# mbitsnbites/himg

Hardware: AMD Instinct MI355X
Metric: Mpixels/s encode+decode, 4K RGBA q=50 (higher is better)
Workload: dtype u8/i16/i32 integer

## Files before the change

### himg_amd/csrc/kernels_dec.hip

```cpp
#include "himg_dev.h"
#include "loop_counts.h"

#include <cstdlib>
#include <type_traits>

namespace himg_dev {

__device__ static constexpr uint8_t kScanD[64] = {
    0,  1,  9,  8,  16, 17, 18, 10, 2,  3,  11, 19, 27, 26, 25, 24,
    32, 33, 34, 35, 36, 28, 20, 12, 4,  5,  13, 21, 29, 37, 45, 44,
    43, 42, 41, 40, 48, 49, 50, 51, 52, 53, 54, 46, 38, 30, 22, 14,
    6,  7,  15, 23, 31, 39, 47, 55, 63, 62, 61, 60, 59, 58, 57, 56};

__device__ static constexpr uint8_t kInvScanD[64] = {
    0, 1, 8, 9, 24, 25, 48, 49, 3, 2, 7, 10, 23, 26, 47, 50, 4, 5, 6, 11, 22, 27, 46, 51, 15, 14, 13, 12, 21, 28, 45, 52, 16, 17, 18, 19, 20, 29, 44, 53, 35, 34, 33, 32, 31, 30, 43, 54, 36, 37, 38, 39, 40, 41, 42, 55, 63, 62, 61, 60, 59, 58, 57, 56};

constexpr int kStGeom = 1, kStUnsupported = 3, kStFormat = 4;
__device__ __host__ constexpr int fmt_err(int stage, int huff) { return kStFormat | (stage << 4) | (huff << 8); }
constexpr int kMaxDepth = 32;
constexpr int kMaxNodes = 2 * kNumSym - 1;
constexpr int kMaxSlow = 128;

__device__ __forceinline__ int clamp255d(int x) { return x < 0 ? 0 : (x > 255 ? 255 : x); }

// ... 1147 lines not shown
      if (__builtin_expect(y == 0, 0)) {
        if ((by >> 31) && tm == TM) {
          ntm = ((1u << (by & 255u)) - 1u) << 3;
          ntb = TB + (((1u << kLutBits) + ((by >> 8) & 0xffffu)) << 3);
          y = (uint32_t)kLutBits | ((uint32_t)kLutBits << 27);
          by = 0;
        } else {
          const int base = tm == TM ? 0 : kLutBits;
          uint32_t len;
          y = walk_token(rd, tb, by, base, &len, &by, &bad);
          adv = len - (uint32_t)base;
        }
      }
      tm = ntm; tbase = ntb;
      const uint32_t extra = __builtin_amdgcn_ubfe((uint32_t)rd.win, y, y >> 5);
      const uint32_t n = y >> 27;
      rd.consume((int)n);
      put(by);
      o += ((y >> 10) & 511u) + extra;
      bp += adv + n;
    };
    while ((int)bp <= limk) step();
    if (tm != TM) step();
    while (bp < lim) {
      uint32_t nbits, cnt, by;
      lean_step<true>(rd, tb, true, &nbits, &cnt, &by, &bad);
      put(by);
      o += cnt;
      bp += nbits;
    }
    rd.retire();
    if (bad) sh->err = 1;
    return;
  }
  for (;;) {
    uint32_t nbits, cnt, by;
    lean_step<true>(rd, tb, exact || (int)bp > limk, &nbits, &cnt, &by, &bad);
    if (exact && (bad || op + cnt > out_size)) { bad = true; break; }
    if (by) {
      if (op + 4 <= op_end) {
        asm volatile("global_store_dword %0, %1, %2" :: "v"((uint32_t)op), "v"(by), "s"(gout) : "memory");
      } else {
#pragma unroll
        for (int j = 0; j < 4; ++j) {
          const uint32_t b = (by >> (8 * j)) & 255u;
          if (b) gout[op + j] = (uint8_t)b;
        }
      }
    }
    op += cnt;
    bp += nbits;
    if (exact && op >= out_size) { sh->endbit = endbit_base + (bp - rel0); break; }
    if (!(bp < lim)) break;
  }
  rd.retire();
  if (bad) sh->err = 1;
}

constexpr uint32_t kTailBits = 48;
struct SubGrid {
  uint32_t b0, lim;
  bool active;
  int last_active;
};
__device__ __forceinline__ SubGrid sub_grid(uint32_t rel0, uint32_t bits, uint32_t sb, int tid) {
  SubGrid q;
  const uint32_t la = (bits - 1u) / sb, L = bits - la * sb;
  const uint32_t S = (L > kTailBits && la + 1u < (uint32_t)kDecThreads) ? sb - (L - kTailBits) : 0u;
  const uint32_t rel_end = rel0 + bits;
  q.b0 = tid ? rel0 + (uint32_t)tid * sb - S : rel0;
  q.lim = rel0 + (uint32_t)(tid + 1) * sb - S;
  if (q.lim > rel_end) q.lim = rel_end;
  q.active = q.b0 < rel_end;
  q.last_active = (int)((bits - 1u + S) / sb);
  return q;
}

struct PreLane {
  uint32_t start, off, nxt, tot, endrel, valid, rounds;
  uint32_t nstart;
};

struct ColdFix { uint32_t start, endpos, cnt, rounds; unsigned long long off, tot; long long c_first; };
__device__ __attribute__((noinline)) ColdFix cold_fixpoint(const uint8_t *p, uint32_t stream_size,
                                                           unsigned long long abs_bit, const uint32_t *grp_lds,
                                                           const uint32_t *nd_lds, StreamShared *sh, bool active,
                                                           uint32_t lim, uint32_t start, uint32_t lead_bits) {
  GrpTables tb;
  tb.grp = reinterpret_cast<const uint2 *>(grp_lds); tb.gx = nullptr; tb.gy = nullptr; tb.nd = nd_lds;
  GReader rd;
  const uint32_t rel0 = rd.attach(p, stream_size, abs_bit);
  ColdFix r;
  r.start = start; r.endpos = start; r.cnt = 0; r.rounds = 0; r.c_first = 0;
  lean_fixpoint(rd, tb, sh, rel0, active, lim, &r.start, &r.endpos, &r.cnt, &r.rounds, false, lead_bits, &r.c_first);
  r.off = block_scan_u64(r.cnt, sh->sm64, &r.tot);
  return r;
}

template <bool FUSED, bool GLOBAL = false, bool PRIMED = false>
__device__ __forceinline__ int decode_stream(const uint8_t *p, uint32_t stream_size, uint32_t pay_off,
                             uint32_t pay_len, uint32_t out_size, const GrpTables &tb,
                             StreamShared *sh, uint8_t *lds_out, uint32_t *win, uint8_t *gout,
                             uint32_t *stats, uint32_t max_sub, uint32_t lead_bits,
                             const uint32_t *pre_start = nullptr, const uint32_t *pre_off = nullptr) {
  const int tid = threadIdx.x;
  if (!PRIMED) {
    if (tid == 0) { sh->err = 0; sh->endbit = ~0ull; }
    __syncthreads();
  }

  const unsigned long long P1 = 8ull * pay_len;
  unsigned long long cur = 0;
  unsigned long long O0 = 0;
  uint32_t st_chunks = 0, st_rounds = 0;
  long long c_sync = 0, c_write = 0, c_r1 = 0, c_t0 = clock64();
  bool synced = false;

  while (cur < P1 && O0 < out_size) {
    synced = false;
    GReader rd;
    const uint32_t rel0 = rd.attach(p, stream_size, 8ull * pay_off + cur);
    ++st_chunks;

    const unsigned long long rem = P1 - cur;
    uint32_t sub = (uint32_t)((rem + kDecThreads - 1) / kDecThreads);
    sub = (sub + 31u) & ~31u;
    sub = sub < kMinSubBits ? kMinSubBits : (sub > max_sub ? max_sub : sub);
    const unsigned long long chunk_bits = (unsigned long long)sub * kDecThreads;
    const uint32_t rel_end = rel0 + (uint32_t)(rem < chunk_bits ? rem : chunk_bits);
    const SubGrid sg = sub_grid(rel0, rel_end - rel0, sub, tid);
    const uint32_t my_b0 = sg.b0, lim = sg.lim;
    const bool active = sg.active;
    const int last_active = sg.last_active;

    uint32_t start = active ? my_b0 : rel_end, endpos = start, cnt = 0;
    unsigned long long tot, off;
    uint32_t wlim = lim;
    const uint32_t pre_valid = cur != 0 ? 0u : pre_off ? pre_off[kDecThreads + 2] : 0u;
    const bool pre = pre_valid != 0, chain = pre_valid == 3u;
    if (pre) {
      const uint32_t ns = tid + 1 < kDecThreads ? pre_start[tid + 1] : ~0u;
      wlim = ns < rel_end - rel0 ? rel0 + ns : rel_end;
    }
    if (pre) {
      start = rel0 + pre_start[tid];
      off = pre_off[tid];
      const uint32_t nxt_off = pre_off[tid + 1];
      cnt = nxt_off - (uint32_t)off;
      tot = pre_off[kDecThreads];
      if (tid == last_active) endpos = rel0 + pre_off[kDecThreads + 1];
      st_rounds += pre_off[kDecThreads + 3];
    } else {
      const ColdFix cf = cold_fixpoint(p, stream_size, 8ull * pay_off + cur, reinterpret_cast<const uint32_t *>(tb.grp),
                                       tb.nd, sh, active, lim, start, lead_bits);
      start = cf.start; endpos = cf.endpos; cnt = cf.cnt; st_rounds += cf.rounds;
      c_r1 += cf.c_first; off = cf.off; tot = cf.tot;
    }
    { const long long t = clock64(); c_sync += t - c_t0; c_t0 = t; }

    const unsigned long long opl = O0 + off;
    const bool inside = opl + cnt < out_size, exact = !inside && opl < out_size;
    if (FUSED) {
      uint32_t end_bp = ~0u;
      if (inside) {
        if (!lean_write(rd, tb, start, wlim, (uint32_t)opl, lds_out, 0u, chain)) sh->err = 1;
      } else if (exact) {
        if (!exact_write(rd, tb, start, wlim, (uint32_t)opl, out_size, lds_out, &end_bp)) sh->err = 1;
      }
      if (end_bp != ~0u) sh->endbit = cur + (end_bp - rel0);
      __syncthreads();
    } else if (GLOBAL) {
      lean_write_global(rd, tb, sh, start, wlim, opl, exact, out_size, cur, rel0, gout, exact ? opl : opl + cnt);
      __syncthreads();
    } else {
      const unsigned long long O1 = (O0 + tot < out_size) ? O0 + tot : out_size;
      lean_write_windows(rd, tb, sh, start, wlim, opl, exact, O0, O1, out_size, cur, rel0, win, gout);
    }
    { const long long t = clock64(); c_write += t - c_t0; c_t0 = t; }

    if (tid == last_active) sh->nxt[0] = endpos;
    __syncthreads();
    const uint32_t last_end = sh->nxt[0];
    cur += (unsigned long long)(last_end - rel0);
    O0 += tot;
    if (last_end == rel0) break;
    __syncthreads();
  }
  if (!synced) __syncthreads();

  int bad = sh->err;
  if (O0 < out_size) bad = 1;
  const unsigned long long E = sh->endbit;
  if (!bad && !(E <= P1 && E + 8 > P1 && E > 0)) bad = 1;
  if (tid == 0 && stats) {
    stats[0] = st_chunks; stats[1] = st_rounds;
    if (!FUSED) { stats[2] = 0; stats[3] = (uint32_t)(c_r1 >> 4); }
    stats[4] = (uint32_t)(c_sync >> 4); stats[5] = (uint32_t)(c_write >> 4);
    stats[6] = pay_len; stats[7] = out_size;
  }
  return bad;
}

__device__ __forceinline__ int decode_row_recorded(const uint8_t *p, uint32_t stream_size, uint32_t pay_off,
                                                   uint32_t pay_len, uint32_t out_size, const GrpTables &tb,
                                                   StreamShared *sh, uint8_t *lds_out, uint32_t *stats,
                                                   const PreLane &pl) {
  const int tid = threadIdx.x;
  const unsigned long long P1 = 8ull * pay_len;
  if (pl.valid == 0 || P1 == 0 || out_size == 0) return -1;
  const long long c_t0 = clock64();
  GReader rd;
  const uint32_t rel0 = rd.attach(p, stream_size, 8ull * pay_off);
  const uint32_t rel_end = rel0 + (uint32_t)P1;
  const uint32_t start = rel0 + pl.start, opl = pl.off, cnt = pl.nxt - pl.off;
  const uint32_t wlim = pl.nstart < (uint32_t)P1 ? rel0 + pl.nstart : rel_end;
  const bool inside = opl + cnt < out_size, exact = !inside && opl < out_size;
  uint32_t end_bp = ~0u;
  if (inside) {
    if (!lean_write(rd, tb, start, wlim, opl, lds_out, 0u, pl.valid == 3u)) sh->err = 1;
  } else if (exact) {
    if (!exact_write(rd, tb, start, wlim, opl, out_size, lds_out, &end_bp)) sh->err = 1;
  }
  if (end_bp != ~0u) sh->endbit = (unsigned long long)(end_bp - rel0);
  __syncthreads();
  const long long c_t1 = clock64();
  int bad = sh->err;
  if (pl.tot < out_size) bad = 1;
  const unsigned long long E = sh->endbit;
  if (!bad && !(E <= P1 && E + 8 > P1 && E > 0)) bad = 1;
  if (tid == 0 && stats) {
    stats[0] = 1; stats[1] = pl.rounds;
    stats[4] = 0; stats[5] = (uint32_t)((c_t1 - c_t0) >> 4);
    stats[6] = pay_len; stats[7] = out_size;
  }
  return bad;
}

// ... 86 lines not shown
  stage_payload(gr, s_pay, (uint32_t)kLresPayWords);
  __syncthreads();
  rd.w = (const __attribute__((address_space(3))) uint32_t *)s_pay;
  rd.jmax = kLresPayWords - 1;
  const unsigned long long rem = P1 - cur;
  const uint32_t rel_end = rel0 + (uint32_t)(rem < (unsigned long long)kLresChunkBits ? rem : kLresChunkBits);
  const uint32_t my_b0 = rel0 + tid * kLresSubBits;
  uint32_t lim = my_b0 + kLresSubBits;
  if (lim > rel_end) lim = rel_end;
  const bool active = my_b0 < rel_end;
  const int last_active = (int)((rel_end - rel0 - 1u) / kLresSubBits);
  uint32_t start = active ? my_b0 : rel_end, endpos = start, cnt = 0, rounds = 0, first = rel0;
  if (FIX) {
    const unsigned long long T = ws.spec_end[slot - 1];
    if (T < cur || T >= cur + kLresSubBits) {
      if (tid == 0) ws.fix_end[slot] = ~0ull;
      return;
    }
    first = rel0 + (uint32_t)(T - cur);
    start = rel0 + ws.spec_start[slot * kDecThreads + tid];
    endpos = rel0 + ws.spec_endpos[slot * kDecThreads + tid];
    cnt = ws.spec_cnt[slot * kDecThreads + tid];
  }
  uint32_t memo[3 * kLresMemo];
  uint32_t *gm = ws.spec_memo + (slot * kDecThreads + tid) * kLresMemo;
#pragma unroll
  for (int e = 0; e < kLresMemo; ++e) {
    memo[3 * e] = ~0u; memo[3 * e + 1] = memo[3 * e + 2] = 0;
    if (FIX && tid > 0) {
      const uint32_t m = gm[e];
      if (m != ~0u) { memo[3 * e] = my_b0 + (m & 63u); memo[3 * e + 1] = lim + ((m >> 6) & 63u); memo[3 * e + 2] = m >> 12; }
    }
  }
  const long long c_in = clock64();
  lean_fixpoint<false, LReader, kLresMemo>(rd, tb, sh, first, active, lim, &start, &endpos, &cnt, &rounds, FIX,
                                           (uint32_t)g.lead_bits, nullptr, nullptr, memo);
  const long long c_fix = clock64() - c_in;
  if (!FIX) {
#pragma unroll
    for (int e = 0; e < kLresMemo; ++e) {
      const uint32_t ds = memo[3 * e] - my_b0, de = memo[3 * e + 1] - lim;
      gm[e] = (memo[3 * e] == ~0u || tid == 0 || ds > 46u || de > 46u || memo[3 * e + 2] >= (1u << 20))
                  ? ~0u : (ds | (de << 6) | (memo[3 * e + 2] << 12));
    }
  }
  unsigned long long tot;
  block_scan_u64(cnt, sh->sm64, &tot);
  ws.spec_start[slot * kDecThreads + tid] = start - rel0;
  ws.spec_endpos[slot * kDecThreads + tid] = endpos - rel0;
  ws.spec_cnt[slot * kDecThreads + tid] = cnt;
  if (tid == last_active) { end_out[slot] = cur + (endpos - rel0); ws.spec_tot[slot] = tot; }
  if (tid == 0) {
    uint32_t *st = ws.stats + ((size_t)f * (g.rows + 1)) * 8;
    atomicAdd(&st[FIX ? 2 : 0], 1u);
    atomicAdd(&st[FIX ? 3 : 1], rounds);
    atomicMax(&st[FIX ? 5 : 4], rounds);
    atomicMax(&st[FIX ? 7 : 6], (uint32_t)(c_fix >> 4));
  }
}

__global__ __launch_bounds__(kDecThreads) void k_lres_spec(Geom g, DecWs ws, const uint8_t *packed,
                                                           size_t in_stride, const uint32_t *sizes) {
  __shared__ LdsTables T;
  __shared__ StreamShared sh;
  __shared__ __attribute__((aligned(16))) uint32_t s_pay[kLresPayWords];
  const int k = blockIdx.x, f = blockIdx.y, tid = threadIdx.x;
  DecFrame *df = ws.frames + f;
  if (tid == 0) sh.flag = df->status;
  __syncthreads();
  if (sh.flag) return;
  const unsigned long long P1 = 8ull * (df->s[0].chunk_end - df->s[0].payload_off);
  const unsigned long long cur = (unsigned long long)k * kLresChunkBits;
  const size_t slot = (size_t)f * ws.lres_chunks + k;
  if (cur >= P1) {
    if (tid == 0) { ws.spec_end[slot] = cur; ws.spec_tot[slot] = 0; }
    return;
  }
  load_dec_tables(ws, df, f, 0, &T);
  __syncthreads();
  const GrpTables tb = tables_of(&T);
  lres_chain_body<false>(g, ws, packed + (size_t)f * in_stride, sizes[f], df, f, k, tb, &sh, s_pay);
}

__global__ __launch_bounds__(kDecThreads) void k_lres_fix(Geom g, DecWs ws, const uint8_t *packed,
                                                          size_t in_stride, const uint32_t *sizes) {
  __shared__ LdsTables T;
  __shared__ StreamShared sh;
  __shared__ uint8_t s_pending[kDecThreads];
  __shared__ int s_bad;
  __shared__ __attribute__((aligned(16))) uint32_t s_pay[kLresPayWords];
  const int f = blockIdx.x, k = threadIdx.x;
  DecFrame *df = ws.frames + f;
  if (k == 0) { ws.ver_ok[f] = 0; ws.lres_endbit[f] = ~0ull; s_bad = 0; sh.flag = df->status; }
  s_pending[k] = 0;
  __syncthreads();
  if (sh.flag) return;
  const uint32_t pay_off = df->s[0].payload_off;
  const unsigned long long P1 = 8ull * (df->s[0].chunk_end - pay_off);
  const int nact = (int)((P1 + kLresChunkBits - 1) / kLresChunkBits);
  if (nact > ws.lres_chunks || nact > kDecThreads) return;
  load_dec_tables(ws, df, f, 0, &T);
  __syncthreads();
  const GrpTables tb = tables_of(&T);
  const uint8_t *p = packed + (size_t)f * in_stride;
  const size_t slot = (size_t)f * ws.lres_chunks + k;
  const unsigned long long cur = (unsigned long long)k * kLresChunkBits;
  if (k == 0) {
    ws.fix_end[slot] = ws.spec_end[slot];
  } else if (k < nact) {
    const unsigned long long T = ws.spec_end[slot - 1];
    bool settled = false;
    if (T >= cur && T < cur + kLresSubBits) {
      GReader rd;
      const uint32_t rel0 = rd.attach(p, sizes[f], 8ull * pay_off + cur);
      const unsigned long long rem = P1 - cur;
      uint32_t lim = rel0 + kLresSubBits;
      const uint32_t rel_end = rel0 + (uint32_t)(rem < (unsigned long long)kLresChunkBits ? rem : kLresChunkBits);
      if (lim > rel_end) lim = rel_end;
      uint32_t pos, c;
      lean_count(rd, tb, rel0 + (uint32_t)(T - cur), lim, &pos, &c);
      if (pos - rel0 == ws.spec_endpos[slot * kDecThreads]) {
        const unsigned long long oldc = ws.spec_cnt[slot * kDecThreads];
        ws.spec_start[slot * kDecThreads] = (uint32_t)(T - cur);
        ws.spec_cnt[slot * kDecThreads] = c;
        ws.spec_tot[slot] = ws.spec_tot[slot] - oldc + c;
        ws.fix_end[slot] = ws.spec_end[slot];
        settled = true;
        atomicAdd(&ws.stats[((size_t)f * (g.rows + 1)) * 8 + 2], 1u);
      }
    }
    if (!settled) s_pending[k] = 1;
  }
  __syncthreads();
  for (int q = 1; q < nact; ++q) {
    if (!s_pending[q]) continue;
    lres_chain_body<true>(g, ws, p, sizes[f], df, f, q, tb, &sh, s_pay);
    __syncthreads();
  }
  __threadfence_block();
  __syncthreads();
  unsigned long long ntot = 0;
  if (k < nact) {
    ntot = ws.spec_tot[slot];
    if (k + 1 < nact && ws.fix_end[slot] != ws.spec_end[slot]) s_bad = 1;
  }
  unsigned long long tot;
  const unsigned long long base = block_scan_u64(ntot, sh.sm64, &tot);
  if (k < nact) ws.ver_base[slot] = base;
  __syncthreads();
  if (k == 0) ws.ver_ok[f] = (s_bad || g.lres_serial) ? 0 : 1;
}

__global__ __launch_bounds__(kDecThreads) void k_lres_write(Geom g, DecWs ws, const uint8_t *packed,
                                                            size_t in_stride, const uint32_t *sizes) {
  __shared__ LdsTables T;
  __shared__ StreamShared sh;
  const int k = blockIdx.x, f = blockIdx.y, tid = threadIdx.x;
  DecFrame *df = ws.frames + f;
  const size_t slot = (size_t)f * ws.lres_chunks + k;
  const unsigned long long O0 = ws.ver_base[slot];
  const uint32_t start_rel = ws.spec_start[slot * kDecThreads + tid];
  const unsigned long long cnt = ws.spec_cnt[slot * kDecThreads + tid];
  if (tid == 0) sh.flag = df->status ? 1 : (ws.ver_ok[f] ? 0 : 2);
  load_dec_tables(ws, df, f, 0, &T);
  __syncthreads();
  if (sh.flag == 1) return;
  if (sh.flag == 2) {
    if (k != 0) return;
    const GrpTables tb0 = tables_of(&T);
    const uint32_t po = df->s[0].payload_off;
    const int bad = decode_stream<false, true>(packed + (size_t)f * in_stride, sizes[f], po, df->s[0].chunk_end - po,
                                               (uint32_t)g.lres_size, tb0, &sh, nullptr, nullptr,
                                               ws.lres_sym + (size_t)f * ws.lres_stride,
                                               ws.stats + ((size_t)f * (g.rows + 1)) * 8, (uint32_t)g.max_sub,
                                               (uint32_t)g.lead_bits);
    if (bad && tid == 0) atomicMax(&df->status, fmt_err(4, 1));
    return;
  }
  const uint32_t pay_off = df->s[0].payload_off;
  const unsigned long long P1 = 8ull * (df->s[0].chunk_end - pay_off);
  const unsigned long long cur = (unsigned long long)k * kLresChunkBits;
  if (cur >= P1) return;
  const uint32_t out_size = (uint32_t)g.lres_size;
  if (O0 >= out_size) return;
  if (tid == 0) { sh.err = 0; sh.endbit = ~0ull; }
  const GrpTables tb = tables_of(&T);
  GReader rd;
  const uint32_t rel0 = rd.attach(packed + (size_t)f * in_stride, sizes[f], 8ull * pay_off + cur);
  const unsigned long long rem = P1 - cur;
  const uint32_t rel_end = rel0 + (uint32_t)(rem < (unsigned long long)kLresChunkBits ? rem : kLresChunkBits);
  uint32_t lim = rel0 + (tid + 1) * kLresSubBits;
  if (lim > rel_end) lim = rel_end;
  const uint32_t start = rel0 + start_rel;
  __syncthreads();
  unsigned long long tot;
  const unsigned long long off = block_scan_u64(cnt, sh.sm64, &tot);
  const unsigned long long opl = O0 + off;
  const bool exact = !(opl + cnt < out_size) && opl < out_size;
  lean_write_global(rd, tb, &sh, start, lim, opl, exact, out_size, cur, rel0,
                    ws.lres_sym + (size_t)f * ws.lres_stride, exact ? opl : opl + cnt);
  __syncthreads();
  if (tid == 0) {
    if (sh.err) atomicMax(&df->status, fmt_err(4, 1));
    if (sh.endbit != ~0ull) ws.lres_endbit[f] = sh.endbit;
  }
}

__global__ void k_lres_finish(DecWs ws, int batch) {
  const int f = blockIdx.x * blockDim.x + threadIdx.x;
  if (f >= batch) return;
  DecFrame *df = ws.frames + f;
  if (df->status || !ws.ver_ok[f]) return;
  const unsigned long long P1 = 8ull * (df->s[0].chunk_end - df->s[0].payload_off);
  const unsigned long long E = ws.lres_endbit[f];
  if (!(E != ~0ull && E <= P1 && E + 8 > P1 && E > 0)) atomicMax(&df->status, fmt_err(4, 1));
}

__device__ __forceinline__ int predict_d(int s1, int s2, int s3, int p) {
  switch (p) {
    default:
    case 0: return clamp255d((3 * (s2 + s3) - 2 * s1 + 2) >> 2);
    case 1: return s2;
    case 2: return s3;
    case 3: return (s2 + s3 + 1) >> 1;
    case 4: return clamp255d(s2 + s3 - s1);
  }
}

__device__ __forceinline__ void wave_lds_sync() {
  __builtin_amdgcn_fence(__ATOMIC_RELEASE, "wavefront");
  __builtin_amdgcn_wave_barrier();
  __builtin_amdgcn_fence(__ATOMIC_ACQUIRE, "wavefront");
}

constexpr int kUnpredWaves = 4;
__global__ __launch_bounds__(64 * kUnpredWaves) void k_lres_unpredict(Geom g, DecWs ws) {
  __shared__ uint8_t rec_s[kUnpredWaves][4][17][18];
  __shared__ uint8_t dl_s[kUnpredWaves][4][16][16];
  __shared__ int16_t s_lmap[128];
  __shared__ int s_status;
  const int lane = threadIdx.x & 63, wv = threadIdx.x >> 6, b = lane >> 4, dv = lane & 15;
  uint8_t (*rec)[17][18] = rec_s[wv];
  uint8_t (*dl)[16][16] = dl_s[wv];
  const int mu = (blockIdx.x * kUnpredWaves + wv) * 4 + b, mv = blockIdx.y;
  const int f = blockIdx.z / g.C, c = blockIdx.z % g.C;
  const DecFrame *df = ws.frames + f;
  if (threadIdx.x == 0) s_status = df->status;
  if (threadIdx.x < 128) s_lmap[threadIdx.x] = df->lmap[threadIdx.x];
  const uint8_t *in = ws.lres_sym + (size_t)f * ws.lres_stride + (size_t)c * g.chan_size;
  uint8_t *m = ws.low + (size_t)f * ws.plane_stride + (size_t)c * g.rows * g.cols;
  const bool live = mu < g.mcols;
  const int u0 = mu * 16, v0 = mv * 16;
  const int bw = live ? min(16, g.cols - u0) : 0, bh = min(16, g.rows - v0);
  const int pc = live ? (int)in[mv * g.mcols + mu] + 2 : 0;
  const uint8_t *src = in + g.mrows * g.mcols + (size_t)v0 * g.cols + (size_t)bh * u0;
  if (dv < bh) {
#pragma unroll
    for (int k = 0; k < 16; ++k)
      if (k < bw) dl[b][dv][k] = src[dv * bw + k];
  }
  __syncthreads();
  if (s_status) return;
  const bool row_live = dv < bh, up_ok = dv > 0;
  uint8_t *rrow = &rec[b][dv + 1][1];
  const uint8_t *urow = &rec[b][dv][1];
  uint8_t *mrow = m + (size_t)(v0 + dv) * g.cols + u0;
  for (int d = 0; d < 31; ++d) {
    const int du = d - dv;
    const bool active = row_live && du >= 0 && du < bw;
    const int duc = active ? du : 0;
    const int left = rrow[duc - 1], up = urow[duc], ul = urow[duc - 1];
    const bool left_ok = duc > 0;
    const int f = up_ok ? up : (left_ok ? left : 128);
    const int s3 = left_ok ? left : f, s2 = f, s1 = (up_ok && left_ok) ? ul : f;
    const int t = s2 + s3;
    const int p0 = clamp255d((3 * t - 2 * s1 + 2) >> 2), p3 = (t + 1) >> 1, p4 = clamp255d(t - s1);
    const int predicted = pc == 1 ? s2 : pc == 2 ? s3 : pc == 3 ? p3 : pc == 4 ? p4 : p0;
    const int sc = (int8_t)dl[b][dv][duc];
    const int mag = s_lmap[sc < 0 ? (sc == -128 ? 127 : -sc) : sc];
    const int un = sc < 0 ? -mag : mag;
    const int val = clamp255d((int)(int16_t)(predicted + un));
    if (active) {
      rrow[du] = (uint8_t)val;
      mrow[du] = (uint8_t)val;
    }
    wave_lds_sync();
  }
}

__device__ __forceinline__ void iwht8(int &x0, int &x1, int &x2, int &x3, int &x4, int &x5,
                                      int &x6, int &x7) {
  const int a0 = x0 + x4, a1 = x1 + x5, a2 = x2 + x6, a3 = x3 + x7;
  const int a4 = x0 - x4, a5 = x1 - x5, a6 = x2 - x6, a7 = x3 - x7;
  const int b0 = a0 + a2, b1 = a1 + a3, b2 = a0 - a2, b3 = a1 - a3;
  const int b4 = a4 + a6, b5 = a5 + a7, b6 = a4 - a6, b7 = a5 - a7;
  x0 = (int16_t)((b0 + b1) >> 3); x1 = (int16_t)((b4 + b5) >> 3);
  x2 = (int16_t)((b6 + b7) >> 3); x3 = (int16_t)((b2 + b3) >> 3);
  x4 = (int16_t)((b2 - b3) >> 3); x5 = (int16_t)((b6 - b7) >> 3);
// ... 1907 lines not shown
  const uint8_t *low = ws.low + (size_t)f * ws.plane_stride;
  uint8_t *img = sa.out + (size_t)f * ((size_t)sa.h * sa.w * g.C);
  const int ycbcr = df->ycbcr;
#pragma unroll 1
  for (int ul = tid; ul < ww; ul += kDecThreads)
    scaled_tile_store_crop<S>(g, (int)L.seg, S * S * (int)L.seg, sym + 4 + ul, low, s_unmap, s_shift, ycbcr, su0 + ul,
                              r, rr, img);
}

#define HIMG_LAUNCH(name, grid, block, ...)                    \
  do {                                                         \
    prof_begin(prof, #name, stream);                           \
    hipLaunchKernelGGL(name, grid, block, 0, stream, __VA_ARGS__); \
    prof_end(prof, stream);                                    \
  } while (0)

int loop_counts_read_dec(unsigned long long *out) { return loop_counts_read(out); }

constexpr uint32_t kLdsMax = 160u * 1024u;
constexpr uint32_t kRowWindowLds = (uint32_t)sizeof(LdsTables) + 64u + kRowWindow + 2u * kWinGuard + 16u;

bool dec_rows_fit_lds(const Geom &g) { return fused_layout(g.row_block).total <= kLdsMax; }

hipError_t dec_set_kernel_attrs() {
  const void *fused[] = {reinterpret_cast<const void *>(&k_dec_row_fused<512>),
                         reinterpret_cast<const void *>(&k_dec_row_fused<256>),
                         reinterpret_cast<const void *>(&k_dec_row_fused<240>),
                         reinterpret_cast<const void *>(&k_dec_row_fused<-1>),
                         reinterpret_cast<const void *>(&k_dec_row_fused<0>)};
  for (const void *k : fused) {
    hipFuncAttributes fa;
    hipError_t e = hipFuncGetAttributes(&fa, k);
    if (e == hipSuccess)
      e = hipFuncSetAttribute(k, hipFuncAttributeMaxDynamicSharedMemorySize, (int)(kLdsMax - fa.sharedSizeBytes));
    if (e != hipSuccess) return e;
  }
  hipError_t e = hipFuncSetAttribute(reinterpret_cast<const void *>(&k_row_window), hipFuncAttributeMaxDynamicSharedMemorySize,
                                     (int)kRowWindowLds);
  if (e != hipSuccess) return e;
  hipFuncAttributes fa;
  e = hipFuncGetAttributes(&fa, reinterpret_cast<const void *>(&k_dec_region));
  if (e == hipSuccess)
    e = hipFuncSetAttribute(reinterpret_cast<const void *>(&k_dec_region), hipFuncAttributeMaxDynamicSharedMemorySize,
                            (int)(kLdsMax - fa.sharedSizeBytes));
  const void *scaled[] = {reinterpret_cast<const void *>(&k_dec_scaled<4, true>), reinterpret_cast<const void *>(&k_dec_scaled<2, true>),
                          reinterpret_cast<const void *>(&k_dec_scaled<4, false>), reinterpret_cast<const void *>(&k_dec_scaled<2, false>),
                          reinterpret_cast<const void *>(&k_dec_scaled_region<4>), reinterpret_cast<const void *>(&k_dec_scaled_region<2>)};
  for (const void *k : scaled) {
    if (e == hipSuccess) e = hipFuncGetAttributes(&fa, k);
    if (e == hipSuccess)
      e = hipFuncSetAttribute(k, hipFuncAttributeMaxDynamicSharedMemorySize, (int)(kLdsMax - fa.sharedSizeBytes));
  }
  return e;
}

int region_strip_tiles(const Geom &g) {
  const uint32_t fixed = region_layout(g.C, 0).total - region_layout(g.C, 0).seg * 64u * (uint32_t)g.C;
  const uint32_t seg = (kLdsMax - 1024u - fixed) / (64u * (uint32_t)g.C) & ~3u;
  return (int)(seg - 8u);
}

int scaled_strip_tiles(const Geom &g, int scale_log2) {
  const uint32_t nseg = (scale_log2 == 1 ? 16u : 4u) * (uint32_t)g.C;
  const RegionLayout L0 = scale_log2 == 1 ? scaled_layout<4>(g.C, 0) : scaled_layout<2>(g.C, 0);
  const uint32_t fixed = L0.total - L0.seg * nseg;
  const uint32_t seg = (kLdsMax - 1024u - fixed) / nseg & ~3u;
  return (int)(seg - 8u);
}

void launch_rowwalk_only(const Geom &g, const DecWs &ws, const uint8_t *d_packed, size_t in_stride,
                         const uint32_t *d_sizes, hipStream_t stream) {
  hipLaunchKernelGGL(k_dec_rowwalk, dim3(1), dim3(64), 0, stream, g, ws, d_packed, in_stride, d_sizes, 0x7fffffff, 0);
}

void launch_rowwalk_range(const Geom &g, const DecWs &ws, const uint8_t *d_packed, size_t in_stride,
                          const uint32_t *d_sizes, int row_end, bool resume, hipStream_t stream) {
  hipLaunchKernelGGL(k_dec_rowwalk, dim3(1), dim3(64), 0, stream, g, ws, d_packed, in_stride, d_sizes, row_end, resume ? 1 : 0);
}

static void launch_lres_chain(const Geom &g, const DecWs &ws, int batch, const uint8_t *d_packed, size_t in_stride,
                              const uint32_t *d_sizes, hipStream_t stream, Profiler *prof) {
  HIMG_LAUNCH(k_lres_spec, dim3(ws.lres_chunks, batch), dim3(kDecThreads), g, ws, d_packed, in_stride, d_sizes);
  HIMG_LAUNCH(k_lres_fix, dim3(batch), dim3(kDecThreads), g, ws, d_packed, in_stride, d_sizes);
  HIMG_LAUNCH(k_lres_write, dim3(ws.lres_chunks, batch), dim3(kDecThreads), g, ws, d_packed,
              in_stride, d_sizes);
  HIMG_LAUNCH(k_lres_finish, dim3((batch + 63) / 64), dim3(64), ws, batch);
  HIMG_LAUNCH(k_lres_unpredict, dim3((g.mcols + 4 * kUnpredWaves - 1) / (4 * kUnpredWaves), g.mrows, batch * g.C),
              dim3(64 * kUnpredWaves), g, ws);
}

static void launch_zero(const Geom &g, const DecWs &ws, int batch, hipStream_t stream, Profiler *prof) {
  const uint32_t n16 = (uint32_t)(((size_t)batch * ws.lres_stride + 15) / 16);
  const uint32_t ns = (uint32_t)((size_t)batch * (g.rows + 1) * 8), nr = ws.rc_stats ? (uint32_t)((size_t)batch * g.rows * 8) : 0u;
  prof_begin(prof, "memset", stream);
  hipLaunchKernelGGL(k_dec_zero, dim3((n16 + 256 * 4 - 1) / (256 * 4)), dim3(256), 0, stream,
                     reinterpret_cast<uint4 *>(ws.lres_sym), n16, ws.stats, ns, ws.rc_stats, nr);
  prof_end(prof, stream);
}

struct CountRule { bool wave; int rpc; Geom g; };
static CountRule count_rule(const Geom &g, long long all_rows, bool one_record) {
  CountRule c = {g.count_wave >= 0 ? g.count_wave != 0 : all_rows >= 8192,
                 all_rows <= 512 ? 1 : all_rows <= 1024 ? 2 : kRowsPerCount, g};
  if (one_record) c.g.max_sub = 0x7fffffff;
  return c;
}

void launch_preview(const Geom &g, const DecWs &ws, int batch, const uint8_t *d_packed, size_t in_stride,
                    const uint32_t *d_sizes, uint32_t *d_head_sizes, uint8_t *d_out, int32_t *d_status,
                    hipStream_t stream, Profiler *prof) {
  launch_zero(g, ws, batch, stream, prof);
  HIMG_LAUNCH(k_dec_parse_head, dim3(batch), dim3(kParseThreads), g, ws, d_packed, in_stride, d_sizes, d_head_sizes);
  launch_lres_chain(g, ws, batch, d_packed, in_stride, d_head_sizes, stream, prof);
  const uint32_t npix = (uint32_t)g.rows * (uint32_t)g.cols;
  HIMG_LAUNCH(k_lres_preview, dim3((npix + 1023u) / 1024u, batch), dim3(256), g, ws, d_out);
  HIMG_LAUNCH(k_dec_status, dim3((batch + 63) / 64), dim3(64), ws, d_status, batch);
}

struct WindowExtents { int nrows = 0, ntiles = 0; long long all_rows = 0; bool stop_early = false; };
static WindowExtents window_extents(const Geom &g, int batch, const int32_t *h_org, int S, int w, int h) {
  WindowExtents e;
  const int F = 8 / S;
  for (int f = 0; f < batch; ++f) {
    const int x = h_org[2 * f] / F, y = h_org[2 * f + 1] / F;
    const int r0 = y / S, r1 = (y + h + S - 1) / S, nt = (x + w + S - 1) / S - x / S;
    e.nrows = r1 - r0 > e.nrows ? r1 - r0 : e.nrows;
    e.ntiles = nt > e.ntiles ? nt : e.ntiles;
    e.stop_early |= r1 < g.rows;
    e.all_rows += r1 - r0;
  }
  return e;
}

void launch_region(const Geom &g, const DecWs &ws_in, int batch, const uint8_t *d_packed, size_t in_stride,
                   const uint32_t *d_sizes, const uint32_t *d_row_index, const int32_t *h_org, const int32_t *d_org,
                   int scale_log2, int w, int h, uint8_t *d_out, int32_t *d_status, hipStream_t stream, Profiler *prof,
                   const DecStreams *ds) {
  DecWs ws = ws_in;
  ws.lane_q = nullptr;
  const int F = 1 << scale_log2, hf = F * h;
  const WindowExtents e = window_extents(g, batch, h_org, 8 / F, w, h);
  launch_zero(g, ws, batch, stream, prof);
  hipStream_t ws_ = ds ? ds->side : stream;
  if (ds) {
    (void)hipEventRecord(ds->ev_fork, stream);
    (void)hipStreamWaitEvent(ws_, ds->ev_fork, 0);
  }
  prof_begin(prof, d_row_index ? "k_region_set_index" : "k_region_rowwalk", ws_);
  if (d_row_index)
    hipLaunchKernelGGL(k_region_set_index, dim3(batch), dim3(256), 0, ws_, g, ws, d_row_index, d_sizes, d_org, hf);
  else
    hipLaunchKernelGGL(k_region_rowwalk, dim3(batch), dim3(64), 0, ws_, g, ws, d_packed, in_stride, d_sizes, d_org, hf);
  prof_end(prof, ws_);
  if (ds) (void)hipEventRecord(ds->ev_walk[0], ws_);
  HIMG_LAUNCH(k_dec_parse, dim3(batch), dim3(kParseThreads), g, ws, d_packed, in_stride, d_sizes);
  launch_lres_chain(g, ws, batch, d_packed, in_stride, d_sizes, stream, prof);
  if (ds) (void)hipStreamWaitEvent(stream, ds->ev_walk[0], 0);
  if (!d_row_index && e.stop_early)
    HIMG_LAUNCH(k_region_walk_end, dim3((batch + 63) / 64), dim3(64), g, ws, d_packed, in_stride, d_org, hf, batch);
  const CountRule cr = count_rule(g, e.all_rows, true);
  if (cr.wave) {
    HIMG_LAUNCH(k_region_count_w, dim3((e.nrows + kCountRowsW - 1) / kCountRowsW, batch), dim3(kDecThreads), cr.g, ws,
                d_packed, in_stride, d_sizes, d_org, hf);
  } else {
    HIMG_LAUNCH(k_region_count, dim3((e.nrows + cr.rpc - 1) / cr.rpc, batch), dim3(kDecThreads), cr.g, ws, d_packed,
                in_stride, d_sizes, d_org, hf, cr.rpc);
  }
  const int smax = scale_log2 ? scaled_strip_tiles(g, scale_log2) : region_strip_tiles(g);
  const int nstrip = (e.ntiles + smax - 1) / smax, sw = (e.ntiles + nstrip - 1) / nstrip;
// ... 233 lines not shown
```

Baseline: 99670.

## Split rare lres refix and serial fallback into separate lean kernels

Moves the rare re-chaining of unsettled chunks out of k_lres_fix into a new k_lres_refix kernel, and the serial decode fallback out of k_lres_write into a new k_lres_serial kernel that also does the end-bit check. The common-path kernels lose big shared buffers and heavy code paths, which should cut their LDS and register use and raise occupancy. The cold fixpoint is force-inlined in the GLOBAL instantiation. In exchange there is one extra kernel launch per decode, and pending state is passed between kernels through global sentinel values.

```diff
diff --git a/himg_amd/csrc/kernels_dec.hip b/himg_amd/csrc/kernels_dec.hip
--- a/himg_amd/csrc/kernels_dec.hip
+++ b/himg_amd/csrc/kernels_dec.hip
@@ -1253,10 +1253,10 @@
 };
 
 struct ColdFix { uint32_t start, endpos, cnt, rounds; unsigned long long off, tot; long long c_first; };
-__device__ __attribute__((noinline)) ColdFix cold_fixpoint(const uint8_t *p, uint32_t stream_size,
-                                                           unsigned long long abs_bit, const uint32_t *grp_lds,
-                                                           const uint32_t *nd_lds, StreamShared *sh, bool active,
-                                                           uint32_t lim, uint32_t start, uint32_t lead_bits) {
+__device__ __forceinline__ ColdFix cold_fixpoint_body(const uint8_t *p, uint32_t stream_size,
+                                                      unsigned long long abs_bit, const uint32_t *grp_lds,
+                                                      const uint32_t *nd_lds, StreamShared *sh, bool active,
+                                                      uint32_t lim, uint32_t start, uint32_t lead_bits) {
   GrpTables tb;
   tb.grp = reinterpret_cast<const uint2 *>(grp_lds); tb.gx = nullptr; tb.gy = nullptr; tb.nd = nd_lds;
   GReader rd;
@@ -1266,6 +1266,12 @@
   lean_fixpoint(rd, tb, sh, rel0, active, lim, &r.start, &r.endpos, &r.cnt, &r.rounds, false, lead_bits, &r.c_first);
   r.off = block_scan_u64(r.cnt, sh->sm64, &r.tot);
   return r;
+}
+__device__ __attribute__((noinline)) ColdFix cold_fixpoint(const uint8_t *p, uint32_t stream_size,
+                                                           unsigned long long abs_bit, const uint32_t *grp_lds,
+                                                           const uint32_t *nd_lds, StreamShared *sh, bool active,
+                                                           uint32_t lim, uint32_t start, uint32_t lead_bits) {
+  return cold_fixpoint_body(p, stream_size, abs_bit, grp_lds, nd_lds, sh, active, lim, start, lead_bits);
 }
 
 template <bool FUSED, bool GLOBAL = false, bool PRIMED = false>
@@ -1322,8 +1328,11 @@
       if (tid == last_active) endpos = rel0 + pre_off[kDecThreads + 1];
       st_rounds += pre_off[kDecThreads + 3];
     } else {
-      const ColdFix cf = cold_fixpoint(p, stream_size, 8ull * pay_off + cur, reinterpret_cast<const uint32_t *>(tb.grp),
-                                       tb.nd, sh, active, lim, start, lead_bits);
+      const uint32_t *grp_lds = reinterpret_cast<const uint32_t *>(tb.grp);
+      const ColdFix cf = GLOBAL ? cold_fixpoint_body(p, stream_size, 8ull * pay_off + cur, grp_lds, tb.nd, sh, active, lim,
+                                                     start, lead_bits)
+                                : cold_fixpoint(p, stream_size, 8ull * pay_off + cur, grp_lds, tb.nd, sh, active, lim, start,
+                                                lead_bits);
       start = cf.start; endpos = cf.endpos; cnt = cf.cnt; st_rounds += cf.rounds;
       c_r1 += cf.c_first; off = cf.off; tot = cf.tot;
     }
@@ -1576,17 +1585,34 @@
   lres_chain_body<false>(g, ws, packed + (size_t)f * in_stride, sizes[f], df, f, k, tb, &sh, s_pay);
 }
 
+
+constexpr int32_t kVerPending = 2;
+constexpr unsigned long long kFixPending = ~0ull - 1ull;
+
+__device__ __forceinline__ void lres_verify(const Geom &g, const DecWs &ws, int f, int nact, StreamShared *sh,
+                                            int *s_bad) {
+  const int k = threadIdx.x;
+  const size_t slot = (size_t)f * ws.lres_chunks + k;
+  unsigned long long ntot = 0;
+  if (k < nact) {
+    ntot = ws.spec_tot[slot];
+    if (k + 1 < nact && ws.fix_end[slot] != ws.spec_end[slot]) *s_bad = 1;
+  }
+  unsigned long long tot;
+  const unsigned long long base = block_scan_u64(ntot, sh->sm64, &tot);
+  if (k < nact) ws.ver_base[slot] = base;
+  __syncthreads();
+  if (k == 0) ws.ver_ok[f] = (*s_bad || g.lres_serial) ? 0 : 1;
+}
+
 __global__ __launch_bounds__(kDecThreads) void k_lres_fix(Geom g, DecWs ws, const uint8_t *packed,
                                                           size_t in_stride, const uint32_t *sizes) {
   __shared__ LdsTables T;
   __shared__ StreamShared sh;
-  __shared__ uint8_t s_pending[kDecThreads];
-  __shared__ int s_bad;
-  __shared__ __attribute__((aligned(16))) uint32_t s_pay[kLresPayWords];
+  __shared__ int s_bad, s_any;
   const int f = blockIdx.x, k = threadIdx.x;
   DecFrame *df = ws.frames + f;
-  if (k == 0) { ws.ver_ok[f] = 0; ws.lres_endbit[f] = ~0ull; s_bad = 0; sh.flag = df->status; }
-  s_pending[k] = 0;
+  if (k == 0) { ws.ver_ok[f] = 0; ws.lres_endbit[f] = ~0ull; s_bad = 0; s_any = 0; sh.flag = df->status; }
   __syncthreads();
   if (sh.flag) return;
   const uint32_t pay_off = df->s[0].payload_off;
@@ -1623,9 +1649,35 @@
         atomicAdd(&ws.stats[((size_t)f * (g.rows + 1)) * 8 + 2], 1u);
       }
     }
-    if (!settled) s_pending[k] = 1;
-  }
-  __syncthreads();
+    if (!settled) { ws.fix_end[slot] = kFixPending; s_any = 1; }
+  }
+  __syncthreads();
+  if (s_any) {
+    if (k == 0) ws.ver_ok[f] = kVerPending;
+    return;
+  }
+  lres_verify(g, ws, f, nact, &sh, &s_bad);
+}
+
+__global__ __launch_bounds__(kDecThreads, 7) void k_lres_refix(Geom g, DecWs ws, const uint8_t *packed,
+                                                               size_t in_stride, const uint32_t *sizes) {
+  __shared__ LdsTables T;
+  __shared__ StreamShared sh;
+  __shared__ uint8_t s_pending[kDecThreads];
+  __shared__ int s_bad;
+  __shared__ __attribute__((aligned(16))) uint32_t s_pay[kLresPayWords];
+  const int f = blockIdx.x, k = threadIdx.x;
+  DecFrame *df = ws.frames + f;
+  if (k == 0) { s_bad = 0; sh.flag = df->status ? 1 : (ws.ver_ok[f] == kVerPending ? 0 : 1); }
+  __syncthreads();
+  if (sh.flag) return;
+  const unsigned long long P1 = 8ull * (df->s[0].chunk_end - df->s[0].payload_off);
+  const int nact = (int)((P1 + kLresChunkBits - 1) / kLresChunkBits);
+  s_pending[k] = (k >= 1 && k < nact && ws.fix_end[(size_t)f * ws.lres_chunks + k] == kFixPending) ? 1 : 0;
+  load_dec_tables(ws, df, f, 0, &T);
+  __syncthreads();
+  const GrpTables tb = tables_of(&T);
+  const uint8_t *p = packed + (size_t)f * in_stride;
   for (int q = 1; q < nact; ++q) {
     if (!s_pending[q]) continue;
     lres_chain_body<true>(g, ws, p, sizes[f], df, f, q, tb, &sh, s_pay);
@@ -1633,16 +1685,7 @@
   }
   __threadfence_block();
   __syncthreads();
-  unsigned long long ntot = 0;
-  if (k < nact) {
-    ntot = ws.spec_tot[slot];
-    if (k + 1 < nact && ws.fix_end[slot] != ws.spec_end[slot]) s_bad = 1;
-  }
-  unsigned long long tot;
-  const unsigned long long base = block_scan_u64(ntot, sh.sm64, &tot);
-  if (k < nact) ws.ver_base[slot] = base;
-  __syncthreads();
-  if (k == 0) ws.ver_ok[f] = (s_bad || g.lres_serial) ? 0 : 1;
+  lres_verify(g, ws, f, nact, &sh, &s_bad);
 }
 
 __global__ __launch_bounds__(kDecThreads) void k_lres_write(Geom g, DecWs ws, const uint8_t *packed,
@@ -1655,22 +1698,10 @@
   const unsigned long long O0 = ws.ver_base[slot];
   const uint32_t start_rel = ws.spec_start[slot * kDecThreads + tid];
   const unsigned long long cnt = ws.spec_cnt[slot * kDecThreads + tid];
-  if (tid == 0) sh.flag = df->status ? 1 : (ws.ver_ok[f] ? 0 : 2);
+  if (tid == 0) sh.flag = (df->status || ws.ver_ok[f] != 1) ? 1 : 0;
   load_dec_tables(ws, df, f, 0, &T);
   __syncthreads();
-  if (sh.flag == 1) return;
-  if (sh.flag == 2) {
-    if (k != 0) return;
-    const GrpTables tb0 = tables_of(&T);
-    const uint32_t po = df->s[0].payload_off;
-    const int bad = decode_stream<false, true>(packed + (size_t)f * in_stride, sizes[f], po, df->s[0].chunk_end - po,
-                                               (uint32_t)g.lres_size, tb0, &sh, nullptr, nullptr,
-                                               ws.lres_sym + (size_t)f * ws.lres_stride,
-                                               ws.stats + ((size_t)f * (g.rows + 1)) * 8, (uint32_t)g.max_sub,
-                                               (uint32_t)g.lead_bits);
-    if (bad && tid == 0) atomicMax(&df->status, fmt_err(4, 1));
-    return;
-  }
+  if (sh.flag) return;
   const uint32_t pay_off = df->s[0].payload_off;
   const unsigned long long P1 = 8ull * (df->s[0].chunk_end - pay_off);
   const unsigned long long cur = (unsigned long long)k * kLresChunkBits;
@@ -1700,14 +1731,33 @@
   }
 }
 
-__global__ void k_lres_finish(DecWs ws, int batch) {
-  const int f = blockIdx.x * blockDim.x + threadIdx.x;
-  if (f >= batch) return;
+__global__ __launch_bounds__(kDecThreads, 7) void k_lres_serial(Geom g, DecWs ws, const uint8_t *packed,
+                                                                size_t in_stride, const uint32_t *sizes) {
+  __shared__ LdsTables T;
+  __shared__ StreamShared sh;
+  const int f = blockIdx.x, tid = threadIdx.x;
   DecFrame *df = ws.frames + f;
-  if (df->status || !ws.ver_ok[f]) return;
-  const unsigned long long P1 = 8ull * (df->s[0].chunk_end - df->s[0].payload_off);
-  const unsigned long long E = ws.lres_endbit[f];
-  if (!(E != ~0ull && E <= P1 && E + 8 > P1 && E > 0)) atomicMax(&df->status, fmt_err(4, 1));
+  if (tid == 0) {
+    const int flag = df->status ? 1 : (ws.ver_ok[f] == 1 ? 0 : 2);
+    sh.flag = flag;
+    if (flag == 0) {
+      const unsigned long long P1 = 8ull * (df->s[0].chunk_end - df->s[0].payload_off);
+      const unsigned long long E = ws.lres_endbit[f];
+      if (!(E != ~0ull && E <= P1 && E + 8 > P1 && E > 0)) atomicMax(&df->status, fmt_err(4, 1));
+    }
+  }
+  __syncthreads();
+  if (sh.flag != 2) return;
+  load_dec_tables(ws, df, f, 0, &T);
+  __syncthreads();
+  const GrpTables tb = tables_of(&T);
+  const uint32_t po = df->s[0].payload_off;
+  const int bad = decode_stream<false, true>(packed + (size_t)f * in_stride, sizes[f], po, df->s[0].chunk_end - po,
+                                             (uint32_t)g.lres_size, tb, &sh, nullptr, nullptr,
+                                             ws.lres_sym + (size_t)f * ws.lres_stride,
+                                             ws.stats + ((size_t)f * (g.rows + 1)) * 8, (uint32_t)g.max_sub,
+                                             (uint32_t)g.lead_bits);
+  if (bad && tid == 0) atomicMax(&df->status, fmt_err(4, 1));
 }
 
 __device__ __forceinline__ int predict_d(int s1, int s2, int s3, int p) {
@@ -3781,9 +3831,10 @@
                               const uint32_t *d_sizes, hipStream_t stream, Profiler *prof) {
   HIMG_LAUNCH(k_lres_spec, dim3(ws.lres_chunks, batch), dim3(kDecThreads), g, ws, d_packed, in_stride, d_sizes);
   HIMG_LAUNCH(k_lres_fix, dim3(batch), dim3(kDecThreads), g, ws, d_packed, in_stride, d_sizes);
+  HIMG_LAUNCH(k_lres_refix, dim3(batch), dim3(kDecThreads), g, ws, d_packed, in_stride, d_sizes);
   HIMG_LAUNCH(k_lres_write, dim3(ws.lres_chunks, batch), dim3(kDecThreads), g, ws, d_packed,
               in_stride, d_sizes);
-  HIMG_LAUNCH(k_lres_finish, dim3((batch + 63) / 64), dim3(64), ws, batch);
+  HIMG_LAUNCH(k_lres_serial, dim3(batch), dim3(kDecThreads), g, ws, d_packed, in_stride, d_sizes);
   HIMG_LAUNCH(k_lres_unpredict, dim3((g.mcols + 4 * kUnpredWaves - 1) / (4 * kUnpredWaves), g.mrows, batch * g.C),
               dim3(64 * kUnpredWaves), g, ws);
 }
```

Result: no change. 99130 (-0.5%).
